# cerbos/cerbos

Hardware: AMD Instinct MI355X
Metric: CheckResources decisions/sec at batch=1M; p50 per-decision us (higher is better)
Workload: dtype u32 ids + f64 attributes (CEL int64/uint64/double)

## Files before the change

### cerbos_amd/csrc/cbh_check_flat.h

```cpp
#pragma once
#include "cbh_check_wave.h"

#define CBH_FLAT_MAX_DEPTH 16
#if defined(CBH_FLAT_WAVES_OVERRIDE)
#define CBH_FLAT_WAVES CBH_FLAT_WAVES_OVERRIDE
#elif !defined(CBH_HOSTSIM)
#define CBH_FLAT_WAVES 4u
#else
#define CBH_FLAT_WAVES 1u
#endif
#define CBH_FLAT_THREADS (CBH_FLAT_WAVES * CBH_BLOCK)

__device__ __forceinline__ u64 wave_or64(u64 v, u32 wave, u32 lane) {
  __shared__ unsigned long long acc[CBH_FLAT_WAVES];
#ifndef CBH_HOSTSIM
  if (lane == 0) __hip_atomic_store(&acc[wave], 0ull, __ATOMIC_RELAXED, __HIP_MEMORY_SCOPE_WORKGROUP);
  (void)wave_ballot(true);
  if (v) (void)__hip_atomic_fetch_or(&acc[wave], (unsigned long long)v, __ATOMIC_RELAXED, __HIP_MEMORY_SCOPE_WORKGROUP);
  (void)wave_ballot(true);
  const u64 r = __hip_atomic_load(&acc[wave], __ATOMIC_RELAXED, __HIP_MEMORY_SCOPE_WORKGROUP);
#else
  if (lane == 0) acc[wave] = 0;
  (void)wave_ballot(true);
  if (v) atomicOr(&acc[wave], (unsigned long long)v);
// ... 367 lines not shown
__device__ __forceinline__ void flat_body(const KernelArgs& ka_regs, Ctx& c, const CrossDev& x = CrossDev{}, const FlatGroupDev& ag = FlatGroupDev{}) {
  static_assert(!CROSS || (COMPACT && !WITH_CALL && !EP), "the direct cross form: compact inputs, no evaluator call, no trail");
  static_assert(!AGROUP || (!COMPACT && !CROSS && !EP), "an action-group launch: the wide inputs, no trail");
  constexpr bool STAGED = MODE == 1;
  constexpr u32 BTYPE = MODE == 2 ? (u32)CBH_B_RESSEG : (u32)CBH_B_RESOURCE;
  const TableDev& t = ka_regs.t;
  const BatchDev& b = ka_regs.b;
  const OutDev& o = ka_regs.o;
  const u32 flags = ka_regs.flags;
  const u32 wave = threadIdx.x / CBH_BLOCK;
#ifdef CBH_PROFILE_CYCLES
  const u64 cyc0 = __builtin_readcyclecounter();
  const u64 rt0 = __builtin_amdgcn_s_memrealtime();
  u32 dbg_rows = 0, dbg_rounds = 0, dbg_evals = 0, dbg_visits = 0;
  u64 cyc_eval = 0, cyc_stage = 0;
#define FLAT_DBG(x) x
#else
#define FLAT_DBG(x)
#endif
  const u32 rix = (CROSS ? 0u : b.req_lo) + blockIdx.x * CBH_FLAT_THREADS + threadIdx.x;
  const bool valid = rix < (CROSS ? x.n_tile : b.req_hi);
  const u32 req = valid ? rix : (CROSS ? 0u : b.req_lo);
  const u32 NR = b.n_requests;
  const u32 w0r = (CROSS ? 0u : b.req_lo) + blockIdx.x * CBH_FLAT_THREADS + wave * CBH_BLOCK;
  const u32 w0 = w0r < (CROSS ? x.n_tile : b.req_hi) ? w0r : (CROSS ? 0u : b.req_lo);
  const u32 wd = valid ? c.tid : 0u;
  const u32 kmax = t.K ? t.K - 1u : 0u;
  u32 pid, kind, r_scope, r_ver, role_off = 0, act_off, role_cnt, act_cnt;
  u32 ac[4], rc[4];
  u32x4u sp{0, 0, 0, 0};
  u32 cls_a0 = 0, cls_r0 = 0;
  bool spec = false; u32 spec_ix = 0;
  u32 x_prow = 0, x_rrow = 0;
  u32 x_done = 0;
  u32 act_total = 0;
  if constexpr (CROSS) {
    const u32 jp = req / x.n, ip = req - jp * x.n;
    x_prow = x.p_order ? x.p_order[ip] : ip;
    x_rrow = x.n + (x.r_order ? x.r_order[x.r_begin + jp] : x.r_begin + jp);
    const u32x4u prec = load_u32x4(b.creq + 4u * (size_t)x_prow), rrec = load_u32x4(b.creq + 4u * (size_t)x_rrow);
    pid = prec.x; kind = rrec.y & 0xFFFFu; r_ver = rrec.y >> 16;
    r_scope = (rrec.z & 0xFFFFu) | (rrec.w & CBH_SCOPE_EXACT);
    role_cnt = valid ? (prec.z >> 16) & 7u : 0u; act_cnt = valid ? (x.act_word >> 20) & 7u : 0u;
#pragma unroll
    for (u32 k = 0; k < 4; ++k) ac[k] = valid ? (x.act_word >> (5u * k)) & 31u : 31u;
    rc[0] = (prec.w >> 20) & 31u; rc[1] = (prec.w >> 25) & 31u; rc[2] = (prec.z >> 22) & 31u; rc[3] = prec.z >> 27;
#pragma unroll
    for (u32 k = 0; k < 4; ++k) rc[k] = valid ? rc[k] : 31u;
    act_off = 0;
    if (x.rg && x.rg->role_group) {
      const u32 rw = x.rg->role_words[x_prow];
      const u32 xa = (x.act_word >> 20) & 7u, word = w0r >> 6;
      u32 prev = 0;
#pragma unroll
      for (u32 k = 0; k < 4; ++k) if (k < xa && w0r < x.n_tile) prev |= ((u32)(x.allow[(size_t)k * x.words + word] >> c.tid) & 1u) << k;
      role_cnt = valid ? (rw >> 20) & 7u : 0u;
#pragma unroll
      for (u32 k = 0; k < 4; ++k) rc[k] = valid ? (rw >> (5u * k)) & 31u : 31u;
      x_done = prev;
      if (wave_ballot(role_cnt != 0 && (((1u << act_cnt) - 1u) & ~prev) != 0) == 0) return;
    }
  } else if constexpr (COMPACT) {
    const u32x4u rec = load_u32x4(b.creq + 4u * (size_t)req);
    pid = rec.x; kind = rec.y & 0xFFFFu; r_ver = rec.y >> 16;
    const u32 w2 = valid ? rec.z : ((rec.z & 0xFFFFu) | 0xFFC00000u), w3 = valid ? rec.w : (rec.w | 0x3FFFFFFFu);
    r_scope = (w2 & 0xFFFFu) | (w3 & CBH_SCOPE_EXACT);
    role_cnt = (w2 >> 16) & 7u; act_cnt = (w2 >> 19) & 7u;
#pragma unroll
    for (u32 k = 0; k < 4; ++k) ac[k] = (w3 >> (5u * k)) & 31u;
    rc[0] = (w3 >> 20) & 31u; rc[1] = (w3 >> 25) & 31u; rc[2] = (w2 >> 22) & 31u; rc[3] = w2 >> 27;
    act_off = 4u * req;
  } else {
#define RQ(f) b.req_u32[(size_t)(f) * NR + req]
  pid = RQ(CBH_RQ_PRINCIPAL_ID); kind = RQ(CBH_RQ_KIND); r_scope = RQ(CBH_RQ_R_SCOPE); r_ver = RQ(CBH_RQ_R_VERSION);
  role_off = RQ(CBH_RQ_ROLE_OFF); act_off = RQ(CBH_RQ_ACT_OFF);
  role_cnt = valid ? RQ(CBH_RQ_ROLE_CNT) : 0; act_cnt = valid ? RQ(CBH_RQ_ACT_CNT) : 0;
#undef RQ
  if constexpr (AGROUP) {
    act_total = act_cnt;
    const u32 g4 = 4u * ag.group, left = act_cnt > g4 ? act_cnt - g4 : 0u;
    act_cnt = left < 4u ? left : 4u; act_off += g4;
  }
  if constexpr (!AGROUP) {
  spec = b.n_tuples >= 4u;
  spec_ix = (4u * req + 4u <= b.n_tuples) ? 4u * req : 0u;
  sp = load_u32x4(spec ? b.tuple_action + spec_ix : b.req_u32);
  }
  const u32 cls_i = threadIdx.x < t.K ? threadIdx.x : kmax;
  cls_a0 = (t.K ? t.action_class : (const CBH_G u8*)b.req_u32)[cls_i]; cls_r0 = (t.K ? t.role_class : (const CBH_G u8*)b.req_u32)[cls_i];
  }
  CcTags cct;
  if constexpr (COMPACT) { for (u32 g = 0; g < CBH_CACHE_COLS / 4; ++g) cct.w[g] = 0; } else cct = cc_load_tags(c, b, NR, w0, wd);
  const bool ptags = COMPACT || (c.flags & CBH_FI_PACKED_TAGS) != 0;
  const u32 all = CROSS ? ((1u << act_cnt) - 1u) & ~x_done : (1u << act_cnt) - 1u;
  const u32 max_depth = t.max_depth < CBH_FLAT_MAX_DEPTH ? t.max_depth : CBH_FLAT_MAX_DEPTH;
  const bool chain8 = t.n_scopes <= 256u;
  const u32 chain_dwords = chain8 ? max_depth * (CBH_BLOCK / 4u) : max_depth * CBH_BLOCK;
  CBH_L u32* chain_si = (CBH_L u32*)cbh_dyn_lds + CBH_FLAT_WAVES * CBH_CC_DWORDS(c.n_cached, ptags) + wave * chain_dwords;
  CBH_L u8* chain_si8 = (CBH_L u8*)chain_si;
  const bool cls_in_lds = t.K <= CBH_FLAT_LDS_STRINGS;
  CBH_L u8* cls_lds = (CBH_L u8*)((CBH_L u32*)cbh_dyn_lds + CBH_FLAT_WAVES * (CBH_CC_DWORDS(c.n_cached, ptags) + chain_dwords));
  u32 aid[4] = {0, 0, 0, 0}, rid[4] = {0, 0, 0, 0};
  if constexpr (!COMPACT) {
#pragma unroll
  for (u32 k = 0; k < 4; ++k) rid[k] = b.roles[k < role_cnt ? role_off + k : 0u];
  const bool spec_hit = spec && act_cnt == 4u && act_off == spec_ix;
  aid[0] = sp.x; aid[1] = sp.y; aid[2] = sp.z; aid[3] = sp.w;
  if (!spec_hit) {
#pragma unroll
    for (u32 k = 0; k < 4; ++k) aid[k] = b.tuple_action[k < act_cnt ? act_off + k : 0u];
  }
  if (cls_in_lds) {
    if (threadIdx.x < t.K) { cls_lds[threadIdx.x] = (u8)cls_a0; cls_lds[t.K + threadIdx.x] = (u8)cls_r0; }
    for (u32 i = threadIdx.x + CBH_FLAT_THREADS; i < t.K; i += CBH_FLAT_THREADS) { cls_lds[i] = t.action_class[i]; cls_lds[t.K + i] = t.role_class[i]; }
  }
  }
  CBH_L u64* segm = (CBH_L u64*)(cls_lds + (cls_in_lds ? ((2u * t.K + 15u) & ~15u) : 0u)) + wave * (CBH_SEG_LDS_BYTES / 8u);
  CBH_L u8* seg_rec = (CBH_L u8*)(segm + 64);
  CBH_L u64* seg_desc = segm + 64 + 16;
  CBH_L u8* lvtab = (CBH_L u8*)(segm + 64 + 16 + 64);
  CBH_L u32* ep_lds = (CBH_L u32*)(cls_lds + (cls_in_lds ? ((2u * t.K + 15u) & ~15u) : 0u) + (MODE == 2 ? CBH_FLAT_WAVES * CBH_SEG_LDS_BYTES : 0u)) + wave * max_depth * 2u * CBH_BLOCK;
  const bool want_ep = EP && (flags & CBH_F_WANT_EFFECTIVE_POLICIES) != 0 && o.eff_pol != nullptr;
  if (EP) { for (u32 d = 0; d < 2u * max_depth; ++d) ep_lds[d * CBH_BLOCK + c.tid] = 0; }
  if constexpr (CROSS) cc_fill_cross(c, b, NR, x_prow, x_rrow, x.side); else if constexpr (COMPACT) cc_fill_compact(c, b, NR, w0, wd); else cc_fill(c, b, NR, w0, wd, cct);
  const bool lenient = (flags & CBH_F_LENIENT_SCOPE_SEARCH) != 0;
  const u32 first_own = chain_first(t, r_scope, FLAG_RES, lenient);
  const u32 first = (AGROUP && ag.group != 0u && act_cnt == 0u) ? CBH_NONE : first_own;
  if constexpr (COMPACT) {
  } else if (cls_in_lds) {
    __syncthreads();
#pragma unroll
    for (u32 k = 0; k < 4; ++k) {
      const u32 ca = cls_lds[aid[k] < t.K ? aid[k] : kmax], cr = cls_lds[t.K + (rid[k] < t.K ? rid[k] : kmax)];
      ac[k] = (k < act_cnt && aid[k] < t.K && ca < 31u) ? ca : 31u;
      rc[k] = (k < role_cnt && rid[k] < t.K && cr < 31u) ? cr : 31u;
    }
  } else {
#pragma unroll
    for (u32 k = 0; k < 4; ++k) {
      const u32 ca = t.action_class[aid[k] < t.K ? aid[k] : kmax], cr = t.role_class[rid[k] < t.K ? rid[k] : kmax];
      ac[k] = (k < act_cnt && aid[k] < t.K && ca < 31u) ? ca : 31u;
      rc[k] = (k < role_cnt && rid[k] < t.K && cr < 31u) ? cr : 31u;
    }
  }
  u32 lane_ac = 0, lane_rc = 0;
  u32 walks = 0;
#pragma unroll
  for (u32 k = 0; k < 4; ++k) {
    if (k < act_cnt) lane_ac |= 1u << ac[k];
    if (k < role_cnt) { lane_rc |= 1u << rc[k]; walks |= all << (4 * k); }
  }
  const u64 wave_cls = wave_or64((u64)lane_ac | ((u64)lane_rc << 32), wave, c.tid);
  const u32 wave_ac = (u32)wave_cls, wave_rc = (u32)(wave_cls >> 32);
  FLAT_DBG(const u64 cyc1 = __builtin_readcyclecounter();)

  Lane L; L.req = req; L.edr = 0; L.status = 0; L.edr_err = false; L.pid = pid;

  u32 S = walks;
  u32 has_allow = 0, allow = 0, deny = 0, err = 0, unsup = 0;
// ... 293 lines not shown
            if (wave_ballot(m != 0) == 0) continue;
            if (EP) touch |= m;
            u32 hit = m;
            if (rw.drcond != CBH_NONE) {
              const u32 how = (rw.flags & CBH_ROW_F_DRLEAF_EMBEDDED) ? 1u : (rw.flags & CBH_ROW_F_DRTREE_EMBEDDED) ? 2u : 0u;
              const u32 lv = leafish_memo(rw.drcond, how, [&] { return uload_rec<LeafRec>(t.rowleaf2, row); }, hit != 0);
              err |= (lv & 2u) ? hit : 0u; unsup |= (lv & 8u) ? hit : 0u;
              hit = (lv & 1u) ? hit : 0u;
            }
            if (rw.cond != CBH_NONE && wave_ballot(hit != 0) != 0) {
              const u32 how = (rw.flags & CBH_ROW_F_LEAF_EMBEDDED) ? 1u : (rw.flags & CBH_ROW_F_TREE_EMBEDDED) ? 2u : 0u;
              const u32 lv = leafish(rw.cond, how, rf.leaf, hit != 0);
              err |= (lv & 2u) ? hit : 0u; unsup |= (lv & 8u) ? hit : 0u;
              hit = (lv & 1u) ? hit : 0u;
            }
            if ((rw.flags & 3u) == CBH_EFFECT_ALLOW) has_allow |= hit;
            else if ((rw.flags & 3u) == CBH_EFFECT_DENY) { deny |= hit; S &= ~hit; }
          }
        }
      }
      if (EP) {
        if (MODE != 2 && have_bucket && bucket.y) g_pol = uload(&t.rows[(size_t)bucket.x * 16u + 3u]);
        if (ing && mydepth < max_depth) { ep_lds[(2u * mydepth) * CBH_BLOCK + c.tid] = touch; ep_lds[(2u * mydepth + 1u) * CBH_BLOCK + c.tid] = g_pol; }
      }
      const u32 ha = ing ? (has_allow & S) : 0u;
      const u32 sp = (uload(&t.scope_flags[g_si]) >> 2) & 3u;
      if (sp == SP_REQUIRE_CONSENT) has_allow &= ~ha;
      else if (sp == SP_OVERRIDE_PARENT) { allow |= ha; S &= ~ha; }
      if (max_depth > 1u) {
        const u32 newly = S_before & ~S;
        dp0 |= (mydepth & 1u) ? newly : 0u; dp1 |= (mydepth & 2u) ? newly : 0u; dp2 |= (mydepth & 4u) ? newly : 0u; dp3 |= (mydepth & 8u) ? newly : 0u;
      }
    }
    const u32 up = uchain_next(t, uload(&t.scope_parent[g_si]), FLAG_RES);
    if (ing) { cur = (mydepth + 1u < max_depth) ? up : CBH_NONE; ++mydepth; }
  }

  FLAT_DBG(const u64 cyc3 = __builtin_readcyclecounter();)
  const bool decided = first == CBH_NONE || !exists;
  const u32 pol_none = (u32)(decided ? CBH_P_NO_MATCH : (role_cnt ? CBH_P_RESOURCE : CBH_P_EMPTY)) << 28 | ((!decided && role_cnt) ? first : 0u);
  const u32 pol_hit = ((u32)CBH_P_RESOURCE << 28) | first;
  const u32 st_ok = (t.flags & CBH_MF_TRACE_ALL) ? CBH_ST_WANTS_TRACE : CBH_ST_OK;
  bool alw[4], won[4];
  u32 sc1[4];
#pragma unroll
  for (u32 k = 0; k < 4; ++k) {
    const u32 ak = allow & (0x1111u << k), dk = deny & (0x1111u << k);
    const u32 sel = ak ? ak : dk;
    const u32 wb = sel & (0u - sel);
    alw[k] = ak != 0; won[k] = sel != 0;
    u32 s = first;
    if (max_depth > 1u) {
      const u32 d = ((dp0 & wb) ? 1u : 0u) | ((dp1 & wb) ? 2u : 0u) | ((dp2 & wb) ? 4u : 0u) | ((dp3 & wb) ? 8u : 0u);
      s = chain8 ? (u32)chain_si8[d * CBH_BLOCK + c.tid] : chain_si[d * CBH_BLOCK + c.tid];
    }
    sc1[k] = (won[k] && k < act_cnt) ? s + 1u : 0u;
  }
  u32 st4 = st_ok * 0x01010101u;
  if (wave_ballot((err | unsup) != 0) != 0) {
    st4 = 0;
#pragma unroll
    for (u32 k = 0; k < 4; ++k) {
      const u32 ak = (allow >> k) & 0x1111u;
      const u32 seen = ak ? (((ak & (0u - ak)) << 1) - 1u) : 0xFFFFu;
      const u32 ek = (err >> k) & 0x1111u & seen, uk = (unsup >> k) & 0x1111u & seen;
      st4 |= (u32)(uk ? CBH_ST_UNSUPPORTED : (ek ? CBH_ST_CEL_ERROR : st_ok)) << (8 * k);
    }
// ... 259 lines not shown
       : fn == cbh_check_flat_kernel_any ? cbh_check_flat_kernel_any_g : fn == cbh_check_flat_kernel_staged ? cbh_check_flat_kernel_staged_g
       : fn == cbh_check_flat_kernel_any_staged ? cbh_check_flat_kernel_any_staged_g : fn == cbh_check_flat_kernel_masks ? cbh_check_flat_kernel_masks_g
       : fn == cbh_check_flat_kernel_any_masks ? cbh_check_flat_kernel_any_masks_g : nullptr;
}
struct FlatGroupStatusArgs { const CBH_G u32* req_u32; const CBH_G u8* dflag; CBH_G u8* status; CBH_G u32* packed; u32 n_requests, lo, hi, pad; };
__global__ __launch_bounds__(256) void cbh_flat_group_status_kernel(FlatGroupStatusArgs a) {
  const u32 r = a.lo + blockIdx.x * 256u + threadIdx.x;
  if (r >= a.hi) return;
  const u32 f = a.dflag[r];
  if (f == 0u) return;
  const size_t NR = a.n_requests;
  const u32 off = a.req_u32[(size_t)CBH_RQ_ACT_OFF * NR + r], cnt = a.req_u32[(size_t)CBH_RQ_ACT_CNT * NR + r];
  for (u32 k = 0; k < cnt; ++k) {
    const u32 w = a.packed ? a.packed[off + k] : 0u;
    const u32 st = a.packed ? cbh_pk_status(w) : (u32)a.status[off + k];
    const u32 now = ((f & 2u) || st == (u32)CBH_ST_UNSUPPORTED) ? (u32)CBH_ST_UNSUPPORTED : (u32)CBH_ST_CEL_ERROR;
    if (a.packed) a.packed[off + k] = (w & ~(3u << 2)) | (now << 2); else if (a.status) a.status[off + k] = (u8)now;
  }
}
struct PkUnpackArgs { CBH_G u8* effect; CBH_G u8* status; CBH_G u32* policy; CBH_G u32* scope; u32 n; u32 bits; };
__global__ __launch_bounds__(256) void cbh_unpack_results_kernel(PkUnpackArgs a) {
  const u32 i = blockIdx.x * 256u + threadIdx.x;
  if (i >= a.n) return;
  const u32 w = a.policy[i];
  a.effect[i] = (u8)cbh_pk_effect(w); a.status[i] = (u8)cbh_pk_status(w);
  a.policy[i] = cbh_pk_policy(w, a.bits); a.scope[i] = cbh_pk_scope(w, a.bits);
}
struct CompactArgs {
  const CBH_G u32* req_u32; const CBH_G u32* roles; const CBH_G u32* tuple_action; const CBH_G u64* col_val;
  const CBH_G u8* action_class; const CBH_G u8* role_class;
  const CBH_G u8* col_tag; CBH_G u32* ctag;
  CBH_G u32* creq; CBH_G u32* cval; CBH_G u32* info;
  u32 n_requests, n_cached, K, narrow;
};
__global__ __launch_bounds__(256) void cbh_compact_scan_kernel(CompactArgs a) {
  const u32 r = blockIdx.x * 256u + threadIdx.x;
  if (r >= a.n_requests) return;
  const size_t NR = a.n_requests;
  u32 m = 0;
  for (u32 k = 0; k < a.n_cached; ++k) m |= (u32)(a.col_val[k * NR + r] >> 32) ? 1u << k : 0u;
#define RQ(f) a.req_u32[(size_t)(f) * NR + r]
  if ((RQ(CBH_RQ_KIND) | RQ(CBH_RQ_R_VERSION) | (RQ(CBH_RQ_R_SCOPE) & ~CBH_SCOPE_EXACT)) >> 16) m |= CBH_CI_MISFIT;
  if (RQ(CBH_RQ_ROLE_CNT) > 4u || RQ(CBH_RQ_ACT_CNT) > 4u) m |= CBH_CI_MISFIT;
  if (RQ(CBH_RQ_ACT_OFF) != 4u * r || RQ(CBH_RQ_ACT_CNT) != 4u) m |= CBH_CI_ACT4;
#undef RQ
#ifdef CBH_HOSTSIM
  a.info[0] |= m;
#else
  if (m & ~__hip_atomic_load(a.info, __ATOMIC_RELAXED, __HIP_MEMORY_SCOPE_AGENT)) atomicOr((unsigned int*)a.info, m);
#endif
}
__global__ __launch_bounds__(256) void cbh_compact_pack_kernel(CompactArgs a) {
  const u32 r = blockIdx.x * 256u + threadIdx.x;
  if (r >= a.n_requests) return;
  const size_t NR = a.n_requests;
#define RQ(f) a.req_u32[(size_t)(f) * NR + r]
  const u32 pid = RQ(CBH_RQ_PRINCIPAL_ID), kind = RQ(CBH_RQ_KIND), r_scope = RQ(CBH_RQ_R_SCOPE), r_ver = RQ(CBH_RQ_R_VERSION);
  const u32 role_off = RQ(CBH_RQ_ROLE_OFF), act_off = RQ(CBH_RQ_ACT_OFF), role_cnt = RQ(CBH_RQ_ROLE_CNT), act_cnt = RQ(CBH_RQ_ACT_CNT);
#undef RQ
  const u32 kmax = a.K ? a.K - 1u : 0u;
  u32 ac[4], rc[4];
  for (u32 k = 0; k < 4; ++k) {
    const u32 aid = a.tuple_action[k < act_cnt ? act_off + k : 0u], rid = a.roles[k < role_cnt ? role_off + k : 0u];
    const u32 ca = a.K ? a.action_class[aid < a.K ? aid : kmax] : 31u, cr = a.K ? a.role_class[rid < a.K ? rid : kmax] : 31u;
    ac[k] = (k < act_cnt && aid < a.K && ca < 31u) ? ca : 31u;
    rc[k] = (k < role_cnt && rid < a.K && cr < 31u) ? cr : 31u;
  }
  CBH_G u32* rec = a.creq + 4u * (size_t)r;
  rec[0] = pid; rec[1] = cbh_creq_w1(kind, r_ver);
  rec[2] = cbh_creq_w2(r_scope, role_cnt, act_cnt, rc[2], rc[3]);
  rec[3] = cbh_creq_w3(r_scope, ac[0], ac[1], ac[2], ac[3], rc[0], rc[1]);
  u32 plane = 0;
  for (u32 k = 0; k < a.n_cached; ++k)
    if ((a.narrow >> k) & 1u) { a.cval[plane * NR + r] = (u32)a.col_val[k * NR + r]; ++plane; }
  for (u32 g = 0; 4u * g < a.n_cached; ++g) {
    u32 w = 0;
    for (u32 j = 0; j < 4u && 4u * g + j < a.n_cached; ++j) w |= (u32)a.col_tag[(4u * g + j) * NR + r] << (8u * j);
    a.ctag[g * NR + r] = w;
  }
}
static inline cbh_check_kernel_fn cbh_flat_compact_variant(cbh_check_kernel_fn fn) {
  return fn == cbh_check_flat_kernel ? cbh_check_flat_kernel_c
       : fn == cbh_check_flat_kernel_staged ? cbh_check_flat_kernel_staged_c : fn == cbh_check_flat_kernel_masks ? cbh_check_flat_kernel_masks_c : nullptr;
}
static inline bool cbh_is_flat_compact_kernel(cbh_check_kernel_fn fn) {
  return fn == cbh_check_flat_kernel_c || fn == cbh_check_flat_kernel_staged_c || fn == cbh_check_flat_kernel_masks_c;
}
__global__ CBH_FLAT_ATTRS(7) void cbh_check_flat_kernel_x(const KernelArgs a, const KernelArgs* __restrict__ ka, const CrossDev x) {
  CBH_FLAT_CTX_C(a, ka);
  flat_body<false, 0, false, false, true, true>(a, c, x);
}
__global__ CBH_FLAT_ATTRS(5) void cbh_check_flat_kernel_staged_x(const KernelArgs a, const KernelArgs* __restrict__ ka, const CrossDev x) {
  CBH_FLAT_CTX_C(a, ka);
  flat_body<false, 1, false, false, true, true>(a, c, x);
}
__global__ CBH_FLAT_ATTRS(4) void cbh_check_flat_kernel_masks_x(const KernelArgs a, const KernelArgs* __restrict__ ka, const CrossDev x) {
  CBH_FLAT_CTX_C(a, ka);
  flat_body<false, 2, false, false, true, true>(a, c, x);
}
__global__ CBH_FLAT_ATTRS(7) void cbh_check_flat_kernel_dr_x(const KernelArgs a, const KernelArgs* __restrict__ ka, const CrossDev x) {
  CBH_FLAT_CTX_C(a, ka);
  flat_body<false, 0, false, true, true, true>(a, c, x);
}
typedef void (*cbh_cross_kernel_fn)(const KernelArgs, const KernelArgs*, const CrossDev);
// ... 59 lines not shown
```

### cerbos_amd/csrc/cbh_check_wave.h

```cpp
#pragma once
#include "cbh_interp.h"

struct RoleSet {
  u32 role; u32 par_off; u32 par_cnt; u64 gbits;
  u64 classes;
};

__device__ __forceinline__ bool roleset_has(const TableDev& t, const RoleSet& rs, u32 pref, u32 globbit) {
  if (globbit && pref == CBH_PAT_ANY) return true;
  if (pref & globbit) return ((rs.gbits >> (pref & 63u)) & 1ull) != 0;
  if (pref == rs.role) return true;
  for (u32 k = 0; k < rs.par_cnt; ++k) if (t.pool[rs.par_off + k] == pref) return true;
  return false;
}

struct __attribute__((aligned(32))) TblRow { u32 flags, cond, drcond, policy, rm_lo, rm_hi, am_lo, am_hi; };
struct LeafRec;
struct __attribute__((aligned(32))) TblRowPat { u32 action, role, resource, counts, a1, a2, r1, r2; };
struct __attribute__((aligned(16))) TblRp { u32 resource, allow_off, allow_cnt, cond; };
struct __attribute__((aligned(16))) TblDr { u32 name, parents_off, parents_cnt, cond; };
struct __attribute__((aligned(32))) TblSlot { u32 k0, k1, k2, k3, v0, v1, v2, v3; };

template <typename R, typename P>
__device__ __forceinline__ R uload_rec(P base, u32 idx) {
// ... 337 lines not shown
    const size_t u = (size_t)kk * NR + req0;
    by[k] = (u32)(base + u)[d];
  }
#pragma unroll
  for (u32 g = 0; g < CBH_CACHE_COLS / 4; ++g) t.w[g] = by[4 * g] | (by[4 * g + 1] << 8) | (by[4 * g + 2] << 16) | (by[4 * g + 3] << 24);
  return t;
}
__device__ __forceinline__ void cc_fill(const Ctx& c, const BatchDev& b, u32 NR, u32 req0, u32 d, const CcTags& t) {
  const bool packed = (c.flags & CBH_FI_PACKED_TAGS) != 0;
  CBH_L u32* tags = c.cc + 2u * c.n_cached * CBH_BLOCK;
  if (packed) {
#pragma unroll
    for (u32 g = 0; g < CBH_CACHE_COLS / 4; ++g) if (4u * g < c.n_cached) tags[g * CBH_BLOCK + c.tid] = t.w[g];
  }
  const u32 d8 = d * 8u;
  for (u32 k = 0; k < c.n_cached; ++k) {
    const size_t u = (size_t)k * NR + req0;
    const CBH_G char* vb = (const CBH_G char*)(b.col_val + u);
    const CBH_G char* vb4 = vb + 4;
    lds_dma_dword(vb + d8, c.cc + k * CBH_BLOCK, c.tid);
    lds_dma_dword(vb4 + d8, c.cc + (c.n_cached + k) * CBH_BLOCK, c.tid);
    if (!packed) {
      const u32 sh = (u32)u & 3u;
#ifndef CBH_HOSTSIM
      const CBH_G char* tb = (const CBH_G char*)(b.col_tag + (u - sh));
      lds_dma_dword(tb + ((d + sh) & ~3u), c.cc + (2 * c.n_cached + k) * CBH_BLOCK, c.tid);
#else
      c.cc[(2 * c.n_cached + k) * CBH_BLOCK + c.tid] = (u32)b.col_tag[u + d] << (((d + sh) & 3u) * 8u);
#endif
    }
  }
}

__device__ __forceinline__ void cc_fill_compact(const Ctx& c, const BatchDev& b, u32 NR, u32 req0, u32 d) {
  const u32 narrow = b.compact_info & CBH_CI_NARROW_MASK;
  CBH_L u32* tags = c.cc + 2u * c.n_cached * CBH_BLOCK;
  for (u32 k = 0; k < c.n_cached; ++k) if ((narrow >> k) & 1u) c.cc[(c.n_cached + k) * CBH_BLOCK + c.tid] = 0u;
  const u32 d4 = d * 4u, d8 = d * 8u;
  for (u32 g = 0; 4u * g < c.n_cached; ++g) {
    const CBH_G char* tb = (const CBH_G char*)(b.ctag + ((size_t)g * NR + req0));
    lds_dma_dword(tb + d4, tags + g * CBH_BLOCK, c.tid);
  }
  u32 plane = 0;
  for (u32 k = 0; k < c.n_cached; ++k) {
    if ((narrow >> k) & 1u) {
      const CBH_G char* vb = (const CBH_G char*)(b.cval + ((size_t)plane * NR + req0));
      lds_dma_dword(vb + d4, c.cc + k * CBH_BLOCK, c.tid);
      ++plane;
    } else {
      const CBH_G char* vb = (const CBH_G char*)(b.col_val + ((size_t)k * NR + req0));
      const CBH_G char* vb4 = vb + 4;
      lds_dma_dword(vb + d8, c.cc + k * CBH_BLOCK, c.tid);
      lds_dma_dword(vb4 + d8, c.cc + (c.n_cached + k) * CBH_BLOCK, c.tid);
    }
  }
}

struct CrossRoleGroup {
  const CBH_G u32* role_words;
  const CBH_G u32* rc_all;
  const CBH_G u32* p_role_cnt;
  u32 role_group;
  u32 open_from;
};
struct CrossDev {
  const CBH_G u32* p_order; const CBH_G u32* r_order;
  CBH_G u64* allow; CBH_G u64* flagged;
  u32 n, r_begin, n_tile, words;
  u32 side;
  u32 act_word;
  const CBH_G struct CrossRoleGroup* rg;
};
__device__ __forceinline__ void cc_fill_cross(const Ctx& c, const BatchDev& b, u32 NR, u32 prow, u32 rrow, u32 side) {
  const u32 narrow = b.compact_info & CBH_CI_NARROW_MASK;
  CBH_L u32* tags = c.cc + 2u * c.n_cached * CBH_BLOCK;
  const u32 have = c.n_cached >= 32u ? 0xFFFFFFFFu : (1u << c.n_cached) - 1u;
  u32 mixed = 0, tp[CBH_CACHE_COLS / 4], tr[CBH_CACHE_COLS / 4];
#pragma unroll
  for (u32 g = 0; g < CBH_CACHE_COLS / 4; ++g) {
    const u32 hg = (have >> (4u * g)) & 0xFu, sg = (side >> (4u * g)) & hg;
    tp[g] = 0; tr[g] = 0;
    if (sg != 0 && sg != hg) {
      mixed |= 1u << g;
      tp[g] = b.ctag[(size_t)g * NR + prow]; tr[g] = b.ctag[(size_t)g * NR + rrow];
    }
  }
#pragma unroll
  for (u32 g = 0; g < CBH_CACHE_COLS / 4; ++g) {
// ... 751 lines not shown
```

### cerbos_amd/csrc/cbh_host_resident.h

```cpp
#pragma once

static bool flat_groups_shape(const cbh_table* t, u32 max_actions, u32 max_roles) {
  return flat_action_groups_on() && !t->reps.empty() && cbh_flat_action_groups(t->reps[0]->dev.n_dr, max_actions, max_roles) != 0;
}
static bool plain_tags_select(const cbh_table* t, u32 max_actions, u32 max_roles) {
  const u32 mf = t->meta[CBH_M_FLAGS];
  return ((mf & CBH_MF_FLAT) && max_roles <= 4 && (max_actions <= 4 || flat_groups_shape(t, max_actions, max_roles))) ||
         ((mf & CBH_MF_WALK2) && t->meta[CBH_M_GSLOTS_ALL] > t->meta[CBH_M_GSLOTS_GENERIC]);
}
static bool has_int_or_container_tag(const uint8_t* p, size_t n) {
  size_t i = 0; uint64_t hit = 0;
  for (; i + 8 <= n; i += 8) {
    uint64_t w; std::memcpy(&w, p + i, 8);
    const uint64_t z = (w & 0xFAFAFAFAFAFAFAFAull) ^ 0x0202020202020202ull;
    hit |= (z - 0x0101010101010101ull) & ~z & 0x8080808080808080ull;
  }
  for (; i < n; ++i) hit |= (uint64_t)((p[i] & 0xFAu) == 0x02u);
  return hit != 0;
}
struct TagRows { size_t first, count; };
template <typename Rows>
static bool sens_tag_hit(const cbh_table* t, const uint8_t* tags, u32 n_columns, size_t n_rows, Rows rows) {
  for (u32 c = 0; c < 32 && c < n_columns; ++c) if ((t->meta[CBH_M_SENS_COLS] >> c) & 1u) {
    const TagRows r = rows(c);
// ... 37 lines not shown
  const u32* role_off = in->req_u32 + (size_t)CBH_RQ_ROLE_OFF * NR; const u32* role_cnt = in->req_u32 + (size_t)CBH_RQ_ROLE_CNT * NR;
  const u32* act_off = in->req_u32 + (size_t)CBH_RQ_ACT_OFF * NR; const u32* act_cnt = in->req_u32 + (size_t)CBH_RQ_ACT_CNT * NR;
  u32 maxa = 0, maxr = 0; u32 bad = 0;
  const u64 n_roles = in->n_roles, n_tuples = in->n_tuples;
  for (size_t r = 0; r < NR; ++r) {
    maxa = act_cnt[r] > maxa ? act_cnt[r] : maxa;
    maxr = role_cnt[r] > maxr ? role_cnt[r] : maxr;
    bad |= (u32)((u64)role_off[r] + role_cnt[r] > n_roles) | (u32)((u64)act_off[r] + act_cnt[r] > n_tuples);
  }
  u32 unordered = 0;
  for (size_t r = 1; r < NR; ++r) unordered |= (u32)((u64)act_off[r] < (u64)act_off[r - 1] + act_cnt[r - 1]);
  u32 wlo = 0xFFFFFFFFu, whi = 0;
  if (maxa > CBH_W2_NA || maxr > CBH_W2_NR)
    for (size_t r = 0; r < NR; ++r)
      if (act_cnt[r] > CBH_W2_NA || role_cnt[r] > CBH_W2_NR) { if (wlo == 0xFFFFFFFFu) wlo = (u32)r; whi = (u32)r + 1; }
  if (maxa > CBH_MAX_ACTIONS_PER_REQUEST) return fail("cbh_batch: a request carries more than CBH_MAX_ACTIONS_PER_REQUEST actions");
  if (bad) return fail("cbh_batch: a request's role or action slice lies outside the batch");
  if (in->n_strings && in->str_off[in->n_strings] > in->str_bytes_len) return fail("cbh_batch: string offsets exceed str_bytes_len");
  sh.max_actions = maxa; sh.max_roles = maxr; sh.ascending = !unordered;
  sh.wide_lo = whi ? wlo : 0; sh.wide_hi = whi;
  sh.table = t; sh.tags = plain_tags_select(t, maxa, maxr) ? in->col_tag : nullptr; sh.n_columns = in->n_columns; sh.n_req = NR;
  sh.plain.store(-1, std::memory_order_relaxed);
  return 0;
}

static bool compact_inputs_on() { static const bool on = env_int("CBH_COMPACT_INPUTS", 1) != 0; return on; }
static int batch_compact(cbh_device_batch* b, hipStream_t s) {
  const TableDev& dev = b->rep->dev;
  BatchDev& d = b->dev;
  if (!compact_inputs_on() || !(dev.flags & CBH_MF_FLAT) || b->shape.max_actions > 4 || b->shape.max_roles > 4 || !d.n_requests) return 0;
  CompactArgs ca{};
  ca.req_u32 = d.req_u32; ca.roles = d.roles; ca.tuple_action = d.tuple_action; ca.col_val = d.col_val; ca.col_tag = d.col_tag;
  ca.action_class = dev.action_class; ca.role_class = dev.role_class; ca.K = dev.K;
  ca.n_requests = d.n_requests; ca.n_cached = d.n_columns < CBH_CACHE_COLS ? d.n_columns : CBH_CACHE_COLS;
  if (dalloc(b, ca.info, 1) != 0) return -1;
  const dim3 grid((d.n_requests + 255u) / 256u);
  u32 info = 0;
  HIPCHK(hipMemsetAsync(ca.info, 0, 4, s));
  hipLaunchKernelGGL(cbh_compact_scan_kernel, grid, dim3(256), 0, s, ca);
  HIPCHK(hipMemcpyAsync(&info, ca.info, 4, hipMemcpyDeviceToHost, s));
  HIPCHK(hipStreamSynchronize(s));
  if (info & CBH_CI_MISFIT) return 0;
  ca.narrow = ~info & ((1u << ca.n_cached) - 1u) & CBH_CI_NARROW_MASK;
  if (dalloc(b, ca.creq, (size_t)4 * d.n_requests) != 0 || dalloc(b, ca.cval, (size_t)__builtin_popcount(ca.narrow) * d.n_requests) != 0 ||
      dalloc(b, ca.ctag, (size_t)((ca.n_cached + 3u) / 4u) * d.n_requests) != 0) return -1;
  hipLaunchKernelGGL(cbh_compact_pack_kernel, grid, dim3(256), 0, s, ca);
  HIPCHK(hipGetLastError());
  d.creq = ca.creq; d.cval = ca.cval; d.ctag = ca.ctag; d.compact_info = ca.narrow | ((info & CBH_CI_ACT4) ? 0u : CBH_CI_ACT4);
  b->compact = true;
  return 0;
}

static int batch_device_buffers(cbh_device_batch* b, size_t gbits_words) {
  BatchDev& d = b->dev; const Replica* rep = b->rep;
  int rc = dalloc(b, d.gbits, gbits_words);
  d.n_gwords = (rep->dev.flags & CBH_MF_WALK2) ? w2_gwords(rep->dev.gslots_generic, rep->dev.gslots_all, b->shape.plain_tags) : 0;
  d.n_gslots = 0;
  if (d.n_gwords) rc |= dalloc(b, d.gres, (size_t)d.n_gwords * d.n_requests); else d.gres = nullptr;
  rc |= dalloc(b, b->out.effect, d.n_tuples);
  rc |= dalloc(b, b->out.policy, d.n_tuples);
  rc |= dalloc(b, b->out.scope, d.n_tuples);
  rc |= dalloc(b, b->out.status, d.n_tuples);
  rc |= dalloc(b, b->out.edr, d.n_requests);
  rc |= dalloc(b, b->d_args, 1);
  return rc;
}
// ... 432 lines not shown
```

### cerbos_amd/csrc/cbh_vm.h

```cpp
#pragma once
#ifndef CBH_HOSTSIM
#include <hip/hip_runtime.h>
#endif
#include <stdint.h>

#include "../../include/cerbos_hip.h"
#include "cbh_blob.h"

typedef uint8_t u8;
typedef uint32_t u32;
typedef uint64_t u64;
typedef int64_t i64;

#define CBH_BLOCK 64
#define CBH_STACK_DEPTH 10
#define CBH_MAX_LOCALS 4
#define CBH_MAX_ITERS 2

#if defined(__HIP_DEVICE_COMPILE__) && !defined(CBH_HOSTSIM)
#define CBH_G __attribute__((address_space(1)))
#define CBH_L __attribute__((address_space(3)))
#else
#define CBH_G
#define CBH_L
// ... 25 lines not shown
  const CBH_G u8* role_class;
  const CBH_G u8* action_class;
  const CBH_G u64* gbits; u32 K;
  const CBH_G u64* nfa[3]; u32 nfa_words[3];
  u32 flags;
  u32 max_depth;
  u32 n_scopes;
  u32 max_bucket;
  const CBH_G u32* segs; const CBH_G u32* leafpool;
  u32 seg_info;
};

struct BatchDev {
  u32 n_requests, n_tuples, n_roles, n_columns, n_strings, heap_len;
  u32 req_lo, req_hi;
  const CBH_G u32* req_u32; const CBH_G u32* roles; const CBH_G u32* tuple_req; const CBH_G u32* tuple_action;
  const CBH_G u8* col_tag; const CBH_G u64* col_val;
  const CBH_G u8* heap_tag; const CBH_G u64* heap_val;
  const CBH_G u32* str_off; const CBH_G u8* str_bytes; const CBH_G u8* str_flags;
  const CBH_G u64* str_keys;
  CBH_G u64* gbits;
  CBH_G u64* gres;
  u32 n_gwords; u32 n_gslots;
  const CBH_G u32* ep_group;
  CBH_G u32* site_cnt; CBH_G u64* site_list; u32 site_cap;
  u32 compact_info;
  const CBH_G u32* creq; const CBH_G u32* cval;
  const CBH_G u32* ctag;
};
#define CBH_CI_NARROW_MASK 0xFFFFu
#define CBH_CI_ACT4 0x10000u
#define CBH_CI_MISFIT 0x20000u
__host__ __device__ __forceinline__ u32 cbh_creq_w1(u32 kind, u32 ver) { return kind | (ver << 16); }
__host__ __device__ __forceinline__ u32 cbh_creq_w2(u32 r_scope, u32 role_cnt, u32 act_cnt, u32 rc2, u32 rc3) {
  return (r_scope & 0xFFFFu) | (role_cnt << 16) | (act_cnt << 19) | (rc2 << 22) | (rc3 << 27);
}
__host__ __device__ __forceinline__ u32 cbh_creq_w3(u32 r_scope, u32 ac0, u32 ac1, u32 ac2, u32 ac3, u32 rc0, u32 rc1) {
  return ac0 | (ac1 << 5) | (ac2 << 10) | (ac3 << 15) | (rc0 << 20) | (rc1 << 25) | (r_scope & 0x80000000u);
}

struct OutDev {
  CBH_G u8* effect; CBH_G u32* policy; CBH_G u32* scope; CBH_G u8* status; CBH_G u64* edr;
  CBH_G u32* trace_rec; CBH_G u32* trace_cnt; u32 trace_cap; u32 ep_words;
  CBH_G u32* eff_pol;
};
#define CBH_PK_MAX_BITS 12u
__host__ __device__ __forceinline__ u32 cbh_pk_bits(u32 n_scopes) { return 32u - (u32)__builtin_clz(n_scopes | 1u); }
__device__ __forceinline__ u32 cbh_pk_word(u32 eff, u32 st, u32 pol, u32 scp, u32 B) {
  return eff | (st << 2) | ((pol >> 28) << 4) | ((pol & 0x0FFFFFFFu) << 7) | ((scp + 1u) << (7u + B));
}
__device__ __forceinline__ u32 cbh_pk_effect(u32 w) { return w & 3u; }
__device__ __forceinline__ u32 cbh_pk_status(u32 w) { return (w >> 2) & 3u; }
__device__ __forceinline__ u32 cbh_pk_policy(u32 w, u32 B) { return ((w >> 4) & 7u) << 28 | ((w >> 7) & ((1u << B) - 1u)); }
__device__ __forceinline__ u32 cbh_pk_scope(u32 w, u32 B) { return (w >> (7u + B)) - 1u; }
__device__ __forceinline__ void ep_mark(const OutDev& o, const BatchDev& b, u32 req, u32 policy) {
  CBH_G u32* w = o.eff_pol + (size_t)(b.ep_group ? b.ep_group[req] : 0u) * o.ep_words + (policy >> 5);
  const u32 bit = 1u << (policy & 31u);
#ifdef CBH_HOSTSIM
  *w |= bit;
#else
  if (!(__hip_atomic_load(w, __ATOMIC_RELAXED, __HIP_MEMORY_SCOPE_AGENT) & bit)) atomicOr((unsigned int*)w, bit);
#endif
}

struct __attribute__((aligned(16))) KernelArgs { TableDev t; BatchDev b; OutDev o; long long now_ns; u32 flags; u32 pad; };

#define CBH_FI_SKIP_WIDE 0x10000u
#define CBH_FI_ONLY_WIDE 0x20000u
#define CBH_FI_ONLY_WIDER 0x40000u
#define CBH_FI_PACKED_TAGS 0x80000u
#define CBH_FI_PACKED_RES 0x100000u
// ... 1036 lines not shown
```

Before: 180.9 billion.

## Precompute first resource scope in compact records and reorder compact column DMA

```diff
diff --git a/cerbos_amd/csrc/cbh_check_flat.h b/cerbos_amd/csrc/cbh_check_flat.h
--- a/cerbos_amd/csrc/cbh_check_flat.h
+++ b/cerbos_amd/csrc/cbh_check_flat.h
@@ -423,6 +423,7 @@
   u32 cls_a0 = 0, cls_r0 = 0;
   bool spec = false; u32 spec_ix = 0;
   u32 x_prow = 0, x_rrow = 0;
+  u32 c_first = CBH_NONE;
   u32 x_done = 0;
   u32 act_total = 0;
   if constexpr (CROSS) {
@@ -431,7 +432,7 @@
     x_rrow = x.n + (x.r_order ? x.r_order[x.r_begin + jp] : x.r_begin + jp);
     const u32x4u prec = load_u32x4(b.creq + 4u * (size_t)x_prow), rrec = load_u32x4(b.creq + 4u * (size_t)x_rrow);
     pid = prec.x; kind = rrec.y & 0xFFFFu; r_ver = rrec.y >> 16;
-    r_scope = (rrec.z & 0xFFFFu) | (rrec.w & CBH_SCOPE_EXACT);
+    r_scope = 0; c_first = cbh_creq_first(rrec.z, rrec.w, (flags & CBH_F_LENIENT_SCOPE_SEARCH) != 0);
     role_cnt = valid ? (prec.z >> 16) & 7u : 0u; act_cnt = valid ? (x.act_word >> 20) & 7u : 0u;
 #pragma unroll
     for (u32 k = 0; k < 4; ++k) ac[k] = valid ? (x.act_word >> (5u * k)) & 31u : 31u;
@@ -452,10 +453,12 @@
       if (wave_ballot(role_cnt != 0 && (((1u << act_cnt) - 1u) & ~prev) != 0) == 0) return;
     }
   } else if constexpr (COMPACT) {
+    static_assert(!EP, "the compact instantiations keep no trail: its LDS stores would have to go in front of the copies");
     const u32x4u rec = load_u32x4(b.creq + 4u * (size_t)req);
+    cc_fill_compact(c, b, NR, w0, wd);
     pid = rec.x; kind = rec.y & 0xFFFFu; r_ver = rec.y >> 16;
     const u32 w2 = valid ? rec.z : ((rec.z & 0xFFFFu) | 0xFFC00000u), w3 = valid ? rec.w : (rec.w | 0x3FFFFFFFu);
-    r_scope = (w2 & 0xFFFFu) | (w3 & CBH_SCOPE_EXACT);
+    r_scope = 0; c_first = cbh_creq_first(w2, w3, (flags & CBH_F_LENIENT_SCOPE_SEARCH) != 0);
     role_cnt = (w2 >> 16) & 7u; act_cnt = (w2 >> 19) & 7u;
 #pragma unroll
     for (u32 k = 0; k < 4; ++k) ac[k] = (w3 >> (5u * k)) & 31u;
@@ -513,9 +516,10 @@
   CBH_L u32* ep_lds = (CBH_L u32*)(cls_lds + (cls_in_lds ? ((2u * t.K + 15u) & ~15u) : 0u) + (MODE == 2 ? CBH_FLAT_WAVES * CBH_SEG_LDS_BYTES : 0u)) + wave * max_depth * 2u * CBH_BLOCK;
   const bool want_ep = EP && (flags & CBH_F_WANT_EFFECTIVE_POLICIES) != 0 && o.eff_pol != nullptr;
   if (EP) { for (u32 d = 0; d < 2u * max_depth; ++d) ep_lds[d * CBH_BLOCK + c.tid] = 0; }
-  if constexpr (CROSS) cc_fill_cross(c, b, NR, x_prow, x_rrow, x.side); else if constexpr (COMPACT) cc_fill_compact(c, b, NR, w0, wd); else cc_fill(c, b, NR, w0, wd, cct);
+  if constexpr (CROSS) cc_fill_cross(c, b, NR, x_prow, x_rrow, x.side); else if constexpr (!COMPACT) cc_fill(c, b, NR, w0, wd, cct);
   const bool lenient = (flags & CBH_F_LENIENT_SCOPE_SEARCH) != 0;
-  const u32 first_own = chain_first(t, r_scope, FLAG_RES, lenient);
+  u32 first_own;
+  if constexpr (COMPACT) first_own = c_first; else first_own = chain_first(t, r_scope, FLAG_RES, lenient);
   const u32 first = (AGROUP && ag.group != 0u && act_cnt == 0u) ? CBH_NONE : first_own;
   if constexpr (COMPACT) {
   } else if (cls_in_lds) {
@@ -875,7 +879,7 @@
         dp0 |= (mydepth & 1u) ? newly : 0u; dp1 |= (mydepth & 2u) ? newly : 0u; dp2 |= (mydepth & 4u) ? newly : 0u; dp3 |= (mydepth & 8u) ? newly : 0u;
       }
     }
-    const u32 up = uchain_next(t, uload(&t.scope_parent[g_si]), FLAG_RES);
+    const u32 up = (COMPACT && max_depth <= 1u) ? CBH_NONE : uchain_next(t, uload(&t.scope_parent[g_si]), FLAG_RES);
     if (ing) { cur = (mydepth + 1u < max_depth) ? up : CBH_NONE; ++mydepth; }
   }
 
@@ -1201,6 +1205,7 @@
   const CBH_G u8* col_tag; CBH_G u32* ctag;
   CBH_G u32* creq; CBH_G u32* cval; CBH_G u32* info;
   u32 n_requests, n_cached, K, narrow;
+  const CBH_G u32* scope_parent; const CBH_G u32* scope_flags; u32 n_scopes;
 };
 __global__ __launch_bounds__(256) void cbh_compact_scan_kernel(CompactArgs a) {
   const u32 r = blockIdx.x * 256u + threadIdx.x;
@@ -1235,10 +1240,18 @@
     ac[k] = (k < act_cnt && aid < a.K && ca < 31u) ? ca : 31u;
     rc[k] = (k < role_cnt && rid < a.K && cr < 31u) ? cr : 31u;
   }
+  const u32 si = r_scope & ~CBH_SCOPE_EXACT;
+  u32 first = CBH_NONE;
+  bool strict = false;
+  if (si < a.n_scopes) {
+    strict = (r_scope & CBH_SCOPE_EXACT) != 0 && (a.scope_flags[si] & FLAG_RES) != 0;
+    first = si;
+    while (first != CBH_NONE && !(a.scope_flags[first] & FLAG_RES)) first = a.scope_parent[first];
+  }
   CBH_G u32* rec = a.creq + 4u * (size_t)r;
   rec[0] = pid; rec[1] = cbh_creq_w1(kind, r_ver);
-  rec[2] = cbh_creq_w2(r_scope, role_cnt, act_cnt, rc[2], rc[3]);
-  rec[3] = cbh_creq_w3(r_scope, ac[0], ac[1], ac[2], ac[3], rc[0], rc[1]);
+  rec[2] = cbh_creq_w2(first, role_cnt, act_cnt, rc[2], rc[3]);
+  rec[3] = cbh_creq_w3(first, strict, ac[0], ac[1], ac[2], ac[3], rc[0], rc[1]);
   u32 plane = 0;
   for (u32 k = 0; k < a.n_cached; ++k)
     if ((a.narrow >> k) & 1u) { a.cval[plane * NR + r] = (u32)a.col_val[k * NR + r]; ++plane; }
diff --git a/cerbos_amd/csrc/cbh_check_wave.h b/cerbos_amd/csrc/cbh_check_wave.h
--- a/cerbos_amd/csrc/cbh_check_wave.h
+++ b/cerbos_amd/csrc/cbh_check_wave.h
@@ -393,28 +393,60 @@
   }
 }
 
+template <typename T> __device__ __forceinline__ T cc_hold(T x) {
+#ifndef CBH_HOSTSIM
+  T y;
+  if constexpr (sizeof(T) == 8) asm volatile("s_mov_b64 %0, %1" : "=s"(y) : "s"(x)); else asm volatile("s_mov_b32 %0, %1" : "=s"(y) : "s"(x));
+  return y;
+#else
+  return x;
+#endif
+}
+__device__ __forceinline__ CBH_L u32* cc_uniform_lds(CBH_L u32* p) {
+#ifndef CBH_HOSTSIM
+  return (CBH_L u32*)(size_t)uniform((u32)(size_t)p);
+#else
+  return p;
+#endif
+}
+template <u32 K>
+__device__ __forceinline__ void cc_cols_compact(CBH_L u32* cc, CBH_L u32* hi, const CBH_G u32* cval, const CBH_G u64* col_val, u32 n, u32 narrow,
+                                                u32 nr, u32 r0, u32 d, u32 plane, u32 tid) {
+  if constexpr (K < CBH_CACHE_COLS) {
+    if (K >= n) return;
+    const bool nb = ((narrow >> K) & 1u) != 0;
+    const u32 sh = nb ? 2u : 3u;
+    const CBH_G char* plane0 = nb ? (const CBH_G char*)(cval + (size_t)plane * nr) : (const CBH_G char*)(col_val + (size_t)K * nr);
+    const CBH_G char* vb = plane0 + ((size_t)r0 << sh);
+    const u32 off = d << sh;
+    lds_dma_dword(vb + off, cc + K * CBH_BLOCK, tid);
+    if (!nb) lds_dma_dword(vb + 4 + off, hi + K * CBH_BLOCK, tid);
+    cc_cols_compact<K + 1>(cc, hi, cval, col_val, n, narrow, nr, r0, d, plane + (nb ? 1u : 0u), tid);
+  }
+}
 __device__ __forceinline__ void cc_fill_compact(const Ctx& c, const BatchDev& b, u32 NR, u32 req0, u32 d) {
-  const u32 narrow = b.compact_info & CBH_CI_NARROW_MASK;
-  CBH_L u32* tags = c.cc + 2u * c.n_cached * CBH_BLOCK;
-  for (u32 k = 0; k < c.n_cached; ++k) if ((narrow >> k) & 1u) c.cc[(c.n_cached + k) * CBH_BLOCK + c.tid] = 0u;
-  const u32 d4 = d * 4u, d8 = d * 8u;
-  for (u32 g = 0; 4u * g < c.n_cached; ++g) {
-    const CBH_G char* tb = (const CBH_G char*)(b.ctag + ((size_t)g * NR + req0));
+  const CBH_G u32* const cval = cc_hold(b.cval); const CBH_G u32* const ctag = cc_hold(b.ctag); const CBH_G u64* const col_val = cc_hold(b.col_val);
+  const u32 n = cc_hold(c.n_cached < CBH_CACHE_COLS ? c.n_cached : CBH_CACHE_COLS);
+  const u32 narrow = cc_hold(b.compact_info & CBH_CI_NARROW_MASK);
+  const u32 nr = cc_hold(NR);
+  const u32 r0 = uniform(req0);
+  CBH_L u32* const cc = cc_uniform_lds(c.cc);
+  CBH_L u32* const hi = cc + n * CBH_BLOCK;
+  CBH_L u32* const tags = cc + 2u * n * CBH_BLOCK;
+  const u32 zero = narrow & ((1u << n) - 1u);
+#pragma unroll
+  for (u32 k = 0; k < CBH_CACHE_COLS; ++k) {
+    if ((zero >> k) == 0u) break;
+    if ((zero >> k) & 1u) hi[k * CBH_BLOCK + c.tid] = 0u;
+  }
+  const u32 d4 = d * 4u;
+#pragma unroll
+  for (u32 g = 0; g < CBH_CACHE_COLS / 4; ++g) {
+    if (4u * g >= n) break;
+    const CBH_G char* tb = (const CBH_G char*)(ctag + ((size_t)g * nr + r0));
     lds_dma_dword(tb + d4, tags + g * CBH_BLOCK, c.tid);
   }
-  u32 plane = 0;
-  for (u32 k = 0; k < c.n_cached; ++k) {
-    if ((narrow >> k) & 1u) {
-      const CBH_G char* vb = (const CBH_G char*)(b.cval + ((size_t)plane * NR + req0));
-      lds_dma_dword(vb + d4, c.cc + k * CBH_BLOCK, c.tid);
-      ++plane;
-    } else {
-      const CBH_G char* vb = (const CBH_G char*)(b.col_val + ((size_t)k * NR + req0));
-      const CBH_G char* vb4 = vb + 4;
-      lds_dma_dword(vb + d8, c.cc + k * CBH_BLOCK, c.tid);
-      lds_dma_dword(vb4 + d8, c.cc + (c.n_cached + k) * CBH_BLOCK, c.tid);
-    }
-  }
+  cc_cols_compact<0>(cc, hi, cval, col_val, n, narrow, nr, r0, d, 0u, c.tid);
 }
 
 struct CrossRoleGroup {
diff --git a/cerbos_amd/csrc/cbh_host_resident.h b/cerbos_amd/csrc/cbh_host_resident.h
--- a/cerbos_amd/csrc/cbh_host_resident.h
+++ b/cerbos_amd/csrc/cbh_host_resident.h
@@ -93,6 +93,7 @@
   CompactArgs ca{};
   ca.req_u32 = d.req_u32; ca.roles = d.roles; ca.tuple_action = d.tuple_action; ca.col_val = d.col_val; ca.col_tag = d.col_tag;
   ca.action_class = dev.action_class; ca.role_class = dev.role_class; ca.K = dev.K;
+  ca.scope_parent = dev.scope_parent; ca.scope_flags = dev.scope_flags; ca.n_scopes = dev.n_scopes;
   ca.n_requests = d.n_requests; ca.n_cached = d.n_columns < CBH_CACHE_COLS ? d.n_columns : CBH_CACHE_COLS;
   if (dalloc(b, ca.info, 1) != 0) return -1;
   const dim3 grid((d.n_requests + 255u) / 256u);
diff --git a/cerbos_amd/csrc/cbh_vm.h b/cerbos_amd/csrc/cbh_vm.h
--- a/cerbos_amd/csrc/cbh_vm.h
+++ b/cerbos_amd/csrc/cbh_vm.h
@@ -81,11 +81,17 @@
 #define CBH_CI_ACT4 0x10000u
 #define CBH_CI_MISFIT 0x20000u
 __host__ __device__ __forceinline__ u32 cbh_creq_w1(u32 kind, u32 ver) { return kind | (ver << 16); }
-__host__ __device__ __forceinline__ u32 cbh_creq_w2(u32 r_scope, u32 role_cnt, u32 act_cnt, u32 rc2, u32 rc3) {
-  return (r_scope & 0xFFFFu) | (role_cnt << 16) | (act_cnt << 19) | (rc2 << 22) | (rc3 << 27);
-}
-__host__ __device__ __forceinline__ u32 cbh_creq_w3(u32 r_scope, u32 ac0, u32 ac1, u32 ac2, u32 ac3, u32 rc0, u32 rc1) {
-  return ac0 | (ac1 << 5) | (ac2 << 10) | (ac3 << 15) | (rc0 << 20) | (rc1 << 25) | (r_scope & 0x80000000u);
+#define CBH_CREQ_FIRST_LENIENT 0x40000000u
+#define CBH_CREQ_FIRST_STRICT 0x80000000u
+__host__ __device__ __forceinline__ u32 cbh_creq_w2(u32 first, u32 role_cnt, u32 act_cnt, u32 rc2, u32 rc3) {
+  return (first != 0xFFFFFFFFu ? first & 0xFFFFu : 0u) | (role_cnt << 16) | (act_cnt << 19) | (rc2 << 22) | (rc3 << 27);
+}
+__host__ __device__ __forceinline__ u32 cbh_creq_w3(u32 first, bool strict, u32 ac0, u32 ac1, u32 ac2, u32 ac3, u32 rc0, u32 rc1) {
+  return ac0 | (ac1 << 5) | (ac2 << 10) | (ac3 << 15) | (rc0 << 20) | (rc1 << 25) | (first != 0xFFFFFFFFu ? CBH_CREQ_FIRST_LENIENT : 0u) |
+         (strict ? CBH_CREQ_FIRST_STRICT : 0u);
+}
+__host__ __device__ __forceinline__ u32 cbh_creq_first(u32 w2, u32 w3, bool lenient) {
+  return (w3 & (lenient ? CBH_CREQ_FIRST_LENIENT : CBH_CREQ_FIRST_STRICT)) ? (w2 & 0xFFFFu) : 0xFFFFFFFFu;
 }
 
 struct OutDev {
```

Measured after the change: 187.1 billion, median of 6. +3.4%, better.
